# YichengDWu/tinyedm

Hardware: AMD Instinct MI355X
Metric: train imgs/sec CIFAR-10 32x32 bf16 (higher is better)
Workload: dtype bf16; 1 GPU; CIFAR-10 32x32 unconditional EDM2 U-Net (conf/cifar10.yaml, 35.6M params) full training step: diffuse+embed+denoiser fwd/bwd+loss+grad all-reduce+Adam+EMA; per_gpu_batch=128, global_batch=128, parallelism=dp1, conditional=False, step_launch=hipGraph replay, collective=none

## Files before the change

### tinyedm_amd/csrc/tail_lowrank.hip

```cpp
#include "common.h"

typedef __attribute__((ext_vector_type(2))) float f32x2;

constexpr size_t LOWRANK_LDS_MAX = 60 * 1024;
static size_t dgrad_lds(int Co, int C, int W, int R, bool fused) {
  const int CL = C / 8, PS = ((256 / CL) * CL) / CL, TP = (W + 3) / 4 * 4 + 4;
  return ((size_t)Co * 9 * C + (size_t)Co * (R + 2) * TP + (fused ? (size_t)PS * C : 0)) * sizeof(float);
}
static size_t wgrad_lds(int Co, int taps, int C, int W, int R) {
  const int halo = taps == 9 ? 1 : 0;
  return ((size_t)Co * taps * C + (size_t)Co * (R + 2 * halo) * (W + 2 * halo)) * sizeof(float);
}
extern "C" int edm_lowrank_supported(int C, int Co, int W, int taps) {
  if (C <= 0 || C % 8 || C > 1024 || Co < 1 || Co > 8 || W <= 0 || (taps != 1 && taps != 9)) return 0;
  if (wgrad_lds(Co, taps, C, W, 1) > LOWRANK_LDS_MAX) return 0;
  return taps == 1 || dgrad_lds(Co, C, W, 1, true) <= LOWRANK_LDS_MAX;
}

__global__ void k_lowrank_df(const float* __restrict__ dD, const float* __restrict__ Fraw,
                             const float* __restrict__ gain_out, const float* __restrict__ sigma, int sstride, float sd,
                             float* __restrict__ dF, float* __restrict__ aux, int CoHW, long n) {
  const float go = *gain_out;
  for (long i = (long)blockIdx.x * blockDim.x + threadIdx.x; i < n; i += (long)gridDim.x * blockDim.x) {
    const int b = (int)(i / CoHW);
    const float s = sigma[b * sstride];
    const float c = s * sd * rsqrtf(s * s + sd * sd);
    const float d = dD[i];
    dF[i] = d * (c * go);
    if (aux) aux[i] = (d * c) * Fraw[i];
  }
}

extern "C" int edm_lowrank_df(const float* dD, const float* Fraw, const float* gain_out, const float* sigma,
                              int sigma_stride, float sigma_data, float* dF, float* aux, int B, int Co, int HW,
                              hipStream_t st) {
  EDM_REQUIRE(dD && gain_out && sigma && dF && (!aux || Fraw), "lowrank_df: null pointer");
  EDM_REQUIRE(B > 0 && HW > 0 && Co >= 1 && Co <= 8 && (sigma_stride == 0 || sigma_stride == 1), "lowrank_df: bad args");
  EDM_REQUIRE((long)Co * HW < (1L << 31), "lowrank_df: sample too large");
  const long n = (long)B * Co * HW;
  const long blocks = (n + 255) / 256;
  hipLaunchKernelGGL(k_lowrank_df, dim3((unsigned)(blocks < 2048 ? blocks : 2048)), dim3(256), 0, st, dD, Fraw, gain_out,
                     sigma, sigma_stride, sigma_data, dF, aux, Co * HW, n);
  EDM_CHECK_LAUNCH("lowrank_df");
  return EDM_OK;
}

template <int CO, bool FUSED>
__global__ __launch_bounds__(256, 4) void k_lowrank_dgrad3x3(const float* __restrict__ dF, const float* __restrict__ Wc,
                                                          float scale, bf16* __restrict__ ga, const bf16* __restrict__ U,
                                                          const float* __restrict__ lin, long lin_stride,
                                                          const float* __restrict__ gain, bf16* __restrict__ gr,
                                                          float* __restrict__ gm, long gm_stride, float pdrop,
                                                          uint32_t seed_lo, uint32_t seed_hi, uint32_t sub, uint32_t step,
                                                          int u_marks, const StepParams* __restrict__ dyn, int H, int W,
                                                          int C, int R, int TP) {
  extern __shared__ __attribute__((aligned(16))) float sm[];
  float* wl = sm;
  float* tl = wl + CO * 9 * C;
  float* red = tl + CO * (R + 2) * TP;
  const int CL = C >> 3;
  const int PS = blockDim.x / CL;
  const int c8 = threadIdx.x % CL, ps = threadIdx.x / CL;
  const int b = blockIdx.y, y0 = blockIdx.x * R;
  const int rows = min(R, H - y0);
  for (int i = threadIdx.x; i < CO * 9 * C / 4; i += blockDim.x)
    reinterpret_cast<f32x4*>(wl)[i] = reinterpret_cast<const f32x4*>(Wc)[i];
  for (int i = threadIdx.x; i < CO * (R + 2) * TP; i += blockDim.x) {
    const int o = i / ((R + 2) * TP), rem = i - o * (R + 2) * TP;
    const int ry = rem / TP, cx = rem - ry * TP;
    const int y = y0 + ry - 1, x = cx - 1;
    float v = 0.f;
    if (y >= 0 && y < H && x >= 0 && x < W) v = dF[(((long)b * CO + o) * H + y) * W + x];
    tl[i] = v;
  }
  __syncthreads();
  ModEpilogue m{};
  float mv[8], part[8];
  if constexpr (FUSED) {
    m.pdrop = pdrop; m.seed_lo = seed_lo; m.seed_hi = seed_hi; m.sub = sub; m.step = step; m.u_marks = u_marks; m.dyn = dyn;
    apply_dyn(m);
    const float g = *gain;
#pragma unroll
    for (int j = 0; j < 8; ++j) {
      mv[j] = lin[(long)b * lin_stride + c8 * 8 + j] * g + 1.0f;
      part[j] = 0.f;
    }
  }
  const int NSX = (W + 3) >> 2;
  const int nstrips = rows * NSX;
  for (int s = ps; s < nstrips; s += PS) {
    const int ry = s / NSX, x0 = (s - ry * NSX) * 4;
    const long p = ((long)b * H + y0 + ry) * W + x0;
    u32x4 ub[4];
    if constexpr (FUSED) {
#pragma unroll
      for (int k = 0; k < 4; ++k) {
        ub[k] = u32x4{0u, 0u, 0u, 0u};
        if (x0 + k < W) ub[k] = *reinterpret_cast<const u32x4*>(U + (p + k) * C + c8 * 8);
      }
    }
    f32x2 acc[4][4];
#pragma unroll
    for (int k = 0; k < 4; ++k)
#pragma unroll
      for (int j = 0; j < 4; ++j) acc[k][j] = f32x2{0.f, 0.f};
#pragma unroll 1
    for (int g = 0; g < 3 * CO; ++g) {
      const int ky = g / CO, o = g - ky * CO;
      {
        const float* tp = tl + (o * (R + 2) + ry + 2 - ky) * TP + x0;
        float dd[6];
#pragma unroll
        for (int j = 0; j < 6; ++j) dd[j] = tp[j];
#pragma unroll
        for (int kx = 0; kx < 3; ++kx) {
          const float* wp = wl + (o * 9 + ky * 3 + kx) * C + c8 * 8;
          const f32x4 w0 = *reinterpret_cast<const f32x4*>(wp), w1 = *reinterpret_cast<const f32x4*>(wp + 4);
          const f32x2 w[4] = {f32x2{w0[0], w0[1]}, f32x2{w0[2], w0[3]}, f32x2{w1[0], w1[1]}, f32x2{w1[2], w1[3]}};
#pragma unroll
          for (int k = 0; k < 4; ++k) {
            const float d = dd[k + 2 - kx];
            const f32x2 d2 = {d, d};
#pragma unroll
            for (int j = 0; j < 4; ++j) acc[k][j] += d2 * w[j];
          }
        }
      }
    }
    u32x4 o8[4];
#pragma unroll
    for (int k = 0; k < 4; ++k) {
      bf16x8 v;
#pragma unroll
      for (int j = 0; j < 4; ++j) {
        v[2 * j] = (bf16)(scale * acc[k][j][0]);
        v[2 * j + 1] = (bf16)(scale * acc[k][j][1]);
      }
      o8[k] = __builtin_bit_cast(u32x4, v);
    }
#pragma unroll
    for (int k = 0; k < 4; ++k) {
      if (x0 + k < W) {
        const long e = (p + k) * C + c8 * 8;
        if (ga) *reinterpret_cast<u32x4*>(ga + e) = o8[k];
        if constexpr (FUSED) *reinterpret_cast<u32x4*>(gr + e) = mod_silu_drop_bwd8(o8[k], ub[k], e >> 3, mv, m, part);
      }
    }
  }
  if constexpr (FUSED) {
#pragma unroll
    for (int j = 0; j < 8; ++j) red[ps * C + c8 * 8 + j] = part[j];
    __syncthreads();
    for (int c = threadIdx.x; c < C; c += blockDim.x) {
      float s = 0.f;
      for (int q = 0; q < PS; ++q) s += red[q * C + c];
      atomicAdd(gm + (long)b * gm_stride + c, s);
    }
  }
}

template <int CO>
static int launch_dgrad(const float* dF, const float* Wc, float scale, void* ga, const void* U, const float* lin,
                        long lin_stride, const float* gain, void* gr, float* gm, long gm_stride, float pdrop,
                        unsigned long long seed, unsigned sub, unsigned step, int u_marked, int B, int H, int W, int C,
                        const void* dyn, hipStream_t st) {
  const int CL = C / 8, block = (256 / CL) * CL, PS = block / CL;
  const int NSX = (W + 3) / 4, TP = NSX * 4 + 4;
  int R = 128 / W;
  R = R < 1 ? 1 : (R > H ? H : R);
  auto lds = [&](int r) { return dgrad_lds(CO, C, W, r, U != nullptr); };
  while (R > 1 && lds(R) > LOWRANK_LDS_MAX) --R;
  EDM_REQUIRE(lds(R) <= LOWRANK_LDS_MAX, "lowrank_dgrad3x3: Co=%d, C=%d, W=%d need %zu bytes of LDS (60 KB at most)", CO, C, W,
              lds(R));
  const dim3 grid((H + R - 1) / R, B);
  if (U)
    hipLaunchKernelGGL((k_lowrank_dgrad3x3<CO, true>), grid, dim3(block), lds(R), st, dF, Wc, scale, (bf16*)ga,
                       (const bf16*)U, lin, lin_stride, gain, (bf16*)gr, gm, gm_stride, pdrop, (uint32_t)seed,
                       (uint32_t)(seed >> 32), sub, step, u_marked, (const StepParams*)dyn, H, W, C, R, TP);
  else
    hipLaunchKernelGGL((k_lowrank_dgrad3x3<CO, false>), grid, dim3(block), lds(R), st, dF, Wc, scale, (bf16*)ga,
                       (const bf16*)nullptr, (const float*)nullptr, 0L, (const float*)nullptr, (bf16*)nullptr,
                       (float*)nullptr, 0L, 0.f, 0u, 0u, 0u, 0u, 0, (const StepParams*)nullptr, H, W, C, R, TP);
  EDM_CHECK_LAUNCH("lowrank_dgrad3x3");
  return EDM_OK;
}

#define EDM_CO_SWITCH(Co, CALL)      \
  switch (Co) {                      \
    case 1: return CALL(1);          \
    case 2: return CALL(2);          \
    case 3: return CALL(3);          \
    case 4: return CALL(4);          \
    case 5: return CALL(5);          \
    case 6: return CALL(6);          \
    case 7: return CALL(7);          \
    default: return CALL(8);         \
  }

extern "C" int edm_lowrank_dgrad3x3(const float* dF, const float* Wc, float scale, void* ga, const void* r1,
                                    const float* lin, long lin_stride, const float* gain, void* gr, float* gm,
                                    long gm_stride, float pdrop, unsigned long long seed, unsigned sub, unsigned step,
                                    int u_marked, int B, int H, int W, int C, int Co, const void* dyn, hipStream_t st) {
  EDM_REQUIRE(dF && Wc && (ga || r1), "lowrank_dgrad3x3: null pointer");
  EDM_REQUIRE(B > 0 && B <= 65535 && H > 0 && W > 0 && C > 0 && C % 8 == 0 && C <= 2048 && Co >= 1 && Co <= 8,
              "lowrank_dgrad3x3: bad args (C %% 8 == 0, Co <= 8 required)");
  EDM_REQUIRE(((uintptr_t)Wc & 15) == 0, "lowrank_dgrad3x3: Wc must be 16-byte aligned");
  if (r1)
    EDM_REQUIRE(lin && gain && gr && gm && lin_stride >= C && gm_stride >= C && pdrop >= 0.f && pdrop < 1.f,
                "lowrank_dgrad3x3: bad modulation-backward args");
#define CALL(CO_) launch_dgrad<CO_>(dF, Wc, scale, ga, r1, lin, lin_stride, gain, gr, gm, gm_stride, pdrop, seed, sub, step, \
                                    u_marked, B, H, W, C, dyn, st)
  EDM_CO_SWITCH(Co, CALL)
#undef CALL
}

template <int CO, int TAPS, int VEC>
__global__ __launch_bounds__(512) void k_lowrank_wgrad(const float* __restrict__ dF, const bf16* __restrict__ X,
                                                       const float* __restrict__ aux, float* __restrict__ ws, int H,
                                                       int W, int C, int R, int upb, int nunits) {
  constexpr int HALO = TAPS == 9 ? 1 : 0, K = TAPS == 9 ? 3 : 1, NB = 8;
  extern __shared__ __attribute__((aligned(16))) float sm[];
  __shared__ float asums[512];
  const int N = CO * TAPS * C, TPW = W + 2 * HALO, TR = R + 2 * HALO;
  float* accl = sm;
  float* tl = sm + N;
  typedef __attribute__((ext_vector_type(VEC / 2))) unsigned int uraw;
  const int CLV = C / VEC;
  const int PS = blockDim.x / CLV;
  const int cv = threadIdx.x % CLV, ps = threadIdx.x / CLV;
  f32x2 acc[CO * TAPS][VEC / 2];
#pragma unroll
  for (int e = 0; e < CO * TAPS; ++e)
#pragma unroll
    for (int h = 0; h < VEC / 2; ++h) acc[e][h] = f32x2{0.f, 0.f};
  float asum = 0.f;
  for (int u = blockIdx.x; u < nunits; u += gridDim.x) {
    const int b = u / upb, y0 = (u - b * upb) * R;
    const int rows = min(R, H - y0);
    __syncthreads();
    for (int i = threadIdx.x; i < CO * TR * TPW; i += blockDim.x) {
      const int o = i / (TR * TPW), rem = i - o * TR * TPW;
      const int ry = rem / TPW, cx = rem - ry * TPW;
      const int y = y0 + ry - HALO, x = cx - HALO;
      float v = 0.f;
      if (y >= 0 && y < H && x >= 0 && x < W)
        v = dF[(((long)b * CO + o) * H + y) * W + x];
      tl[i] = v;
    }
    if (aux) {
      for (int o = 0; o < CO; ++o) {
        const float* ap = aux + (((long)b * CO + o) * H + y0) * W;
        for (int i = threadIdx.x; i < rows * W; i += blockDim.x) asum += ap[i];
      }
    }
    __syncthreads();
    const int np = rows * W;
    const bf16* xp = X + (((long)b * H + y0) * W) * C + cv * VEC;
    int ry = ps / W, x = ps - (ps / W) * W;
    uraw nx[NB];
    auto fetch = [&](int q0) {
#pragma unroll
      for (int i = 0; i < NB; ++i) {
        const int q = q0 + i * PS;
        nx[i] = uraw{};
        if (q < np) nx[i] = *reinterpret_cast<const uraw*>(xp + (long)q * C);
      }
    };
    fetch(ps);
    for (int q0 = ps; q0 < np; q0 += NB * PS) {
      uraw cur[NB];
#pragma unroll
      for (int i = 0; i < NB; ++i) cur[i] = nx[i];
      if (q0 + NB * PS < np) fetch(q0 + NB * PS);
#pragma unroll
      for (int i = 0; i < NB; ++i) {
        if (q0 + i * PS < np) {
          typedef __attribute__((ext_vector_type(VEC))) __bf16 bfv;
          const bfv xv = __builtin_bit_cast(bfv, cur[i]);
          f32x2 xf[VEC / 2];
#pragma unroll
          for (int h = 0; h < VEC / 2; ++h) xf[h] = f32x2{(float)xv[2 * h], (float)xv[2 * h + 1]};
#pragma unroll
          for (int o = 0; o < CO; ++o)
#pragma unroll
            for (int ky = 0; ky < K; ++ky)
#pragma unroll
              for (int kx = 0; kx < K; ++kx) {
                const float d = tl[(o * TR + ry + 2 * HALO - ky) * TPW + x + 2 * HALO - kx];
                const f32x2 d2 = {d, d};
#pragma unroll
                for (int h = 0; h < VEC / 2; ++h) acc[o * TAPS + ky * K + kx][h] += d2 * xf[h];
              }
        }
        x += PS;
        while (x >= W) {
          x -= W;
          ++ry;
        }
      }
    }
  }
  for (int r = 0; r < PS; ++r) {
    __syncthreads();
    if (ps == r) {
#pragma unroll
      for (int e = 0; e < CO * TAPS; ++e) {
#pragma unroll
        for (int h = 0; h < VEC / 2; ++h) {
          f32x2* ap = reinterpret_cast<f32x2*>(accl + e * C + cv * VEC + 2 * h);
          f32x2 v = acc[e][h];
          if (r) v += *ap;
          *ap = v;
        }
      }
    }
  }
  asums[threadIdx.x] = asum;
  __syncthreads();
  float* row = ws + (long)blockIdx.x * (N + 4);
  for (int i = threadIdx.x; i < N; i += blockDim.x) row[i] = accl[i];
  if (threadIdx.x == 0) {
    float s = 0.f;
    for (int i = 0; i < (int)blockDim.x; ++i) s += asums[i];
    row[N] = s;
  }
}

__global__ __launch_bounds__(1024) void k_lowrank_reduce(const float* __restrict__ ws, int nwg, int N, float* __restrict__ G,
                                                         float* __restrict__ aux_out) {
  __shared__ float part[16][64];
  const int l = threadIdx.x & 63, seg = threadIdx.x >> 6;
  const int e = blockIdx.x * 64 + l;
  const int per = (nwg + 15) / 16;
  const int r0 = seg * per;
  float v[16];
#pragma unroll
  for (int k = 0; k < 16; ++k) {
    const int r = r0 + k;
    v[k] = (e <= N && k < per && r < nwg) ? ws[(long)r * (N + 4) + e] : 0.f;
  }
  float s = 0.f;
#pragma unroll
  for (int k = 0; k < 16; ++k) s += v[k];
  part[seg][l] = s;
  __syncthreads();
  if (seg == 0 && e <= N) {
    float t = 0.f;
#pragma unroll
    for (int k = 0; k < 16; ++k) t += part[k][l];
    if (e < N) G[e] = t;
    else if (aux_out) *aux_out += t;
  }
}

template <int CO>
static int launch_wgrad(const float* dF, const void* X, int taps, const float* aux, float* G, float* aux_out, float* ws,
                        long ws_floats, int B, int H, int W, int C, int nwg, hipStream_t st) {
  constexpr int VEC = CO <= 4 ? 4 : 2;
  const int CLV = C / VEC;
  int PS = 512 / CLV;
  PS = PS > 16 ? 16 : PS;
  const int block = PS * CLV, halo = taps == 9 ? 1 : 0;
  const int N = CO * taps * C;
  int R = 512 / W;
  R = R < 1 ? 1 : (R > H ? H : R);
  auto lds = [&](int r) { return wgrad_lds(CO, taps, C, W, r); };
  while (R > 1 && lds(R) > LOWRANK_LDS_MAX) --R;
  EDM_REQUIRE(lds(R) <= LOWRANK_LDS_MAX, "lowrank_wgrad: Co=%d, taps=%d, C=%d, W=%d need %zu bytes of LDS (60 KB at most)", CO,
              taps, C, W, lds(R));
  const int upb = (H + R - 1) / R;
  EDM_REQUIRE((long)B * upb < (1L << 31), "lowrank_wgrad: too many units");
  const int nunits = B * upb;
  const int grid = nunits < nwg ? nunits : nwg;
  EDM_REQUIRE(ws_floats >= (long)grid * (N + 4), "lowrank_wgrad: workspace of %ld floats, %ld needed", ws_floats,
              (long)grid * (N + 4));
  if (taps == 9)
    hipLaunchKernelGGL((k_lowrank_wgrad<CO, 9, VEC>), dim3(grid), dim3(block), lds(R), st, dF, (const bf16*)X, aux, ws, H, W, C,
                       R, upb, nunits);
  else
    hipLaunchKernelGGL((k_lowrank_wgrad<CO, 1, VEC>), dim3(grid), dim3(block), lds(R), st, dF, (const bf16*)X, aux, ws, H, W, C,
                       R, upb, nunits);
  EDM_CHECK_LAUNCH("lowrank_wgrad");
  hipLaunchKernelGGL(k_lowrank_reduce, dim3((N + 1 + 63) / 64), dim3(1024), 0, st, ws, grid, N, G, aux_out);
  EDM_CHECK_LAUNCH("lowrank_reduce");
  return EDM_OK;
}

constexpr int LOWRANK_WGRAD_NWG = 256;
extern "C" long edm_lowrank_wgrad_workspace(int C, int Co, int taps) {
  return (long)LOWRANK_WGRAD_NWG * ((long)Co * taps * C + 4);
}

extern "C" int edm_lowrank_wgrad(const float* dF, const void* X, int taps, const float* aux, float* G, float* aux_out,
                                 float* ws, long ws_floats, int B, int H, int W, int C, int Co, hipStream_t st) {
  EDM_REQUIRE(dF && X && G && ws && (!aux || aux_out), "lowrank_wgrad: null pointer");
  EDM_REQUIRE(B > 0 && H > 0 && W > 0 && C > 0 && C % 8 == 0 && C <= 1024 && Co >= 1 && Co <= 8 && (taps == 1 || taps == 9),
              "lowrank_wgrad: bad args (C %% 8 == 0, Co <= 8, taps 1 or 9 required)");
#define CALL(CO_) launch_wgrad<CO_>(dF, X, taps, aux, G, aux_out, ws, ws_floats, B, H, W, C, LOWRANK_WGRAD_NWG, st)
  EDM_CO_SWITCH(Co, CALL)
#undef CALL
}

__global__ void k_lowrank_expand_wc(const float* __restrict__ wout, const bf16* __restrict__ wd, float* __restrict__ Wc,
                                    int Co, int O, int I, int taps) {
  const int lane = threadIdx.x & 63;
  const int row = blockIdx.x * (blockDim.x >> 6) + (threadIdx.x >> 6);
  if (row >= taps * I) return;
  const int tt = row / I, ci = row - tt * I;
  float acc[8] = {0, 0, 0, 0, 0, 0, 0, 0};
  for (int c = lane * 8; c < O; c += 64 * 8) {
    float v[8];
    load8(wd + (long)row * O + c, v);
#pragma unroll
    for (int o = 0; o < 8; ++o)
      if (o < Co) {
#pragma unroll
        for (int j = 0; j < 8; ++j) acc[o] += wout[(long)o * O + c + j] * v[j];
      }
  }
#pragma unroll
  for (int o = 0; o < 8; ++o)
    if (o < Co) {
      const float s = wave_sum(acc[o]);
      if (lane == 0) Wc[((long)o * taps + (taps - 1 - tt)) * I + ci] = s;
    }
}
extern "C" int edm_lowrank_expand_wc(const float* wout_hat, const void* wd, float* Wc, int Co, int O, int I, int taps,
                                     hipStream_t st) {
  EDM_REQUIRE(wout_hat && wd && Wc, "lowrank_expand_wc: null pointer");
  EDM_REQUIRE(Co >= 1 && Co <= 8 && O > 0 && O % 8 == 0 && I > 0 && taps >= 1, "lowrank_expand_wc: bad args");
  hipLaunchKernelGGL(k_lowrank_expand_wc, dim3((taps * I + 3) / 4), dim3(256), 0, st, wout_hat, (const bf16*)wd, Wc, Co, O,
                     I, taps);
  EDM_CHECK_LAUNCH("lowrank_expand_wc");
  return EDM_OK;
}

__global__ void k_lowrank_expand_slab(const float* __restrict__ wout, const float* __restrict__ G, float* __restrict__ slab,
                                      float scale, int Co, int O, int I, int Ipad, int taps, long n) {
  for (long e = (long)blockIdx.x * blockDim.x + threadIdx.x; e < n; e += (long)gridDim.x * blockDim.x) {
    const int i = (int)(e % Ipad);
    const long tc = e / Ipad;
    const int c = (int)(tc % O), t = (int)(tc / O);
    float s = 0.f;
    if (i < I)
      for (int o = 0; o < Co; ++o) s += wout[(long)o * O + c] * G[((long)o * taps + t) * I + i];
    slab[e] = scale * s;
  }
}
extern "C" int edm_lowrank_expand_slab(const float* wout_hat, const float* G, float* slab, float scale, int Co, int O, int I,
                                       int Ipad, int taps, hipStream_t st) {
  EDM_REQUIRE(wout_hat && G && slab, "lowrank_expand_slab: null pointer");
  EDM_REQUIRE(Co >= 1 && Co <= 8 && O > 0 && I > 0 && Ipad >= I && taps >= 1, "lowrank_expand_slab: bad args");
  const long n = (long)taps * O * Ipad;
  const long blocks = (n + 255) / 256;
  hipLaunchKernelGGL(k_lowrank_expand_slab, dim3((unsigned)(blocks < 4096 ? blocks : 4096)), dim3(256), 0, st, wout_hat, G,
                     slab, scale, Co, O, I, Ipad, taps, n);
  EDM_CHECK_LAUNCH("lowrank_expand_slab");
  return EDM_OK;
}

constexpr int TAIL_LPP = 8;
static size_t tail_fwd_lds(int Co, int C, int Cc, int W, int R) {
  return ((size_t)Co * 9 * C + (size_t)Co * Cc + (size_t)R * W * 10 * Co) * sizeof(float);
}
extern "C" int edm_lowrank_tail_supported(int C, int Cc, int Co, int W) {
  if (C <= 0 || C % 8 || C > 1024 || Cc <= 0 || Cc % 8 || Cc > 2048 || Co < 1 || Co > 8 || W <= 0) return 0;
  return tail_fwd_lds(Co, C, Cc, W, 1) <= LOWRANK_LDS_MAX;
}

template <int CO, int NK, int PX>
__device__ __forceinline__ void tail_dots(const bf16* const (&xp)[PX], int Cx, const float* __restrict__ w, int wso, int lig,
                                          float (&s)[PX][NK * CO]) {
  f32x2 acc[PX][NK * CO];
#pragma unroll
  for (int k = 0; k < PX; ++k)
#pragma unroll
    for (int v = 0; v < NK * CO; ++v) acc[k][v] = f32x2{0.f, 0.f};
  const int CL = Cx >> 3;
  for (int c8 = lig; c8 < CL; c8 += TAIL_LPP) {
    f32x2 xf[PX][4];
#pragma unroll
    for (int k = 0; k < PX; ++k) {
      u32x4 raw = u32x4{0u, 0u, 0u, 0u};
      if (xp[k]) raw = *reinterpret_cast<const u32x4*>(xp[k] + c8 * 8);
      const bf16x8 xv = __builtin_bit_cast(bf16x8, raw);
#pragma unroll
      for (int h = 0; h < 4; ++h) xf[k][h] = f32x2{(float)xv[2 * h], (float)xv[2 * h + 1]};
    }
#pragma unroll
    for (int o = 0; o < CO; ++o)
#pragma unroll
      for (int kk = 0; kk < NK; ++kk) {
        const float* wp = w + (long)(o * wso + kk) * Cx + c8 * 8;
        const f32x4 w0 = *reinterpret_cast<const f32x4*>(wp), w1 = *reinterpret_cast<const f32x4*>(wp + 4);
        const f32x2 wv[4] = {f32x2{w0[0], w0[1]}, f32x2{w0[2], w0[3]}, f32x2{w1[0], w1[1]}, f32x2{w1[2], w1[3]}};
#pragma unroll
        for (int k = 0; k < PX; ++k)
#pragma unroll
          for (int h = 0; h < 4; ++h) acc[k][kk * CO + o] += xf[k][h] * wv[h];
      }
  }
#pragma unroll
  for (int k = 0; k < PX; ++k)
#pragma unroll
    for (int v = 0; v < NK * CO; ++v) s[k][v] = group_sum<TAIL_LPP>(acc[k][v][0] + acc[k][v][1]);
}

template <int CO, int PX>
__global__ __launch_bounds__(512) void k_lowrank_tail_fwd(const bf16* __restrict__ a2, const bf16* __restrict__ cat,
                                                          const float* __restrict__ Wc, const float* __restrict__ Wp,
                                                          float sb, float sa, const float* __restrict__ gain_out,
                                                          const float* __restrict__ noisy, const float* __restrict__ sigma,
                                                          int sstride, float sd, float* __restrict__ D,
                                                          float* __restrict__ Fraw, int H, int W, int C, int Cc, int R) {
  extern __shared__ __attribute__((aligned(16))) float sm[];
  float* wl = sm;
  float* wpl = wl + CO * 9 * C;
  float* pt = wpl + CO * Cc;
  const int RW = R * W;
  float* qt = pt + 3 * RW * 3 * CO;
  const int b = blockIdx.y, y0 = blockIdx.x * R;
  const int rows = min(R, H - y0);
  for (int i = threadIdx.x; i < CO * 9 * C / 4; i += blockDim.x)
    reinterpret_cast<f32x4*>(wl)[i] = reinterpret_cast<const f32x4*>(Wc)[i];
  for (int i = threadIdx.x; i < CO * Cc / 4; i += blockDim.x)
    reinterpret_cast<f32x4*>(wpl)[i] = reinterpret_cast<const f32x4*>(Wp)[i];
  __syncthreads();
  const int lig = threadIdx.x % TAIL_LPP, grp = threadIdx.x / TAIL_LPP, NG = blockDim.x / TAIL_LPP;
#pragma unroll 1
  for (int ky = 0; ky < 3; ++ky) {
    const int r_lo = max(y0 + ky - 1, 0), r_hi = min(y0 + rows - 1 + ky - 1, H - 1);
    const int np = (r_hi - r_lo + 1) * W;
    const int slot0 = (r_lo - (y0 + ky - 1)) * W;
    const bf16* base = a2 + (((long)b * H + r_lo) * W) * C;
    float* po = pt + (long)ky * RW * 3 * CO;
    for (int n0 = grp * PX; n0 < np; n0 += NG * PX) {
      const bf16* xp[PX];
#pragma unroll
      for (int k = 0; k < PX; ++k) xp[k] = n0 + k < np ? base + (long)(n0 + k) * C : nullptr;
      float s[PX][3 * CO];
      tail_dots<CO, 3, PX>(xp, C, wl + ky * 3 * C, 9, lig, s);
#pragma unroll
      for (int k = 0; k < PX; ++k)
        if (n0 + k < np) {
#pragma unroll
          for (int v = 0; v < 3 * CO; ++v)
            if ((v % TAIL_LPP) == lig) po[(long)(slot0 + n0 + k) * 3 * CO + v] = s[k][v];
        }
    }
  }
  {
    const int np = rows * W;
    const bf16* base = cat + (((long)b * H + y0) * W) * Cc;
    for (int n0 = grp * PX; n0 < np; n0 += NG * PX) {
      const bf16* xp[PX];
#pragma unroll
      for (int k = 0; k < PX; ++k) xp[k] = n0 + k < np ? base + (long)(n0 + k) * Cc : nullptr;
      float s[PX][CO];
      tail_dots<CO, 1, PX>(xp, Cc, wpl, 1, lig, s);
#pragma unroll
      for (int k = 0; k < PX; ++k)
        if (n0 + k < np) {
#pragma unroll
          for (int v = 0; v < CO; ++v)
            if ((v % TAIL_LPP) == lig) qt[(long)(n0 + k) * CO + v] = s[k][v];
        }
    }
  }
  __syncthreads();
  const float go = *gain_out;
  const float sg = sigma[b * sstride];
  const float den = sg * sg + sd * sd;
  const float cskip = sd * sd / den, cout = sg * sd * rsqrtf(den);
  for (int i = threadIdx.x; i < CO * rows * W; i += blockDim.x) {
    const int o = i / (rows * W), n = i - o * rows * W;
    const int ry = n / W, x = n - ry * W;
    float s = 0.f;
#pragma unroll
    for (int ky = 0; ky < 3; ++ky) {
      const int iy = y0 + ry + ky - 1;
      if (iy < 0 || iy >= H) continue;
#pragma unroll
      for (int kx = 0; kx < 3; ++kx) {
        const int ix = x + kx - 1;
        if (ix < 0 || ix >= W) continue;
        s += pt[((long)ky * RW + ry * W + ix) * 3 * CO + kx * CO + o];
      }
    }
    const float f = sb * s + sa * qt[(long)n * CO + o];
    const long idx = (((long)b * CO + o) * H + y0 + ry) * W + x;
    if (Fraw) Fraw[idx] = f;
    D[idx] = f * go * cout + noisy[idx] * cskip;
  }
}

template <int CO>
static int launch_tail_fwd(const void* a2, const void* cat, const float* Wc, const float* Wp, float sb, float sa,
                           const float* gain_out, const float* noisy, const float* sigma, int sstride, float sd, float* D,
                           float* Fraw, int B, int H, int W, int C, int Cc, hipStream_t st) {
  constexpr int PX = CO <= 4 ? 2 : 1;
  int R = 128 / W;
  R = R < 1 ? 1 : (R > H ? H : R);
  auto lds = [&](int r) { return tail_fwd_lds(CO, C, Cc, W, r); };
  while (R > 1 && lds(R) > LOWRANK_LDS_MAX) --R;
  EDM_REQUIRE(lds(R) <= LOWRANK_LDS_MAX, "lowrank_tail_fwd: Co=%d, C=%d, Cc=%d, W=%d need %zu bytes of LDS (60 KB at most)", CO,
              C, Cc, W, lds(R));
  const long want = ((long)(R + 1) * W + PX - 1) / PX * TAIL_LPP;
  int block = want >= 512 ? 512 : (int)((want + 63) / 64 * 64);
  const dim3 grid((H + R - 1) / R, B);
  hipLaunchKernelGGL((k_lowrank_tail_fwd<CO, PX>), grid, dim3(block), lds(R), st, (const bf16*)a2, (const bf16*)cat, Wc, Wp, sb,
                     sa, gain_out, noisy, sigma, sstride, sd, D, Fraw, H, W, C, Cc, R);
  EDM_CHECK_LAUNCH("lowrank_tail_fwd");
  return EDM_OK;
}

extern "C" int edm_lowrank_tail_fwd(const void* a2, const void* cat, const float* Wc, const float* Wp, float sb, float sa,
                                    const float* gain_out, const float* noisy, const float* sigma, int sigma_stride,
                                    float sigma_data, float* D, float* Fraw, int B, int H, int W, int C, int Cc, int Co,
                                    hipStream_t st) {
  EDM_REQUIRE(a2 && cat && Wc && Wp && gain_out && noisy && sigma && D, "lowrank_tail_fwd: null pointer");
  EDM_REQUIRE(B > 0 && B <= 65535 && H > 0 && W > 0 && (sigma_stride == 0 || sigma_stride == 1), "lowrank_tail_fwd: bad args");
  EDM_REQUIRE(edm_lowrank_tail_supported(C, Cc, Co, W), "lowrank_tail_fwd: unsupported shape C=%d Cc=%d Co=%d W=%d", C, Cc, Co, W);
  EDM_REQUIRE((((uintptr_t)Wc | (uintptr_t)Wp | (uintptr_t)a2 | (uintptr_t)cat) & 15) == 0,
              "lowrank_tail_fwd: operands must be 16-byte aligned");
#define CALL(CO_) launch_tail_fwd<CO_>(a2, cat, Wc, Wp, sb, sa, gain_out, noisy, sigma, sigma_stride, sigma_data, D, Fraw, B, \
                                       H, W, C, Cc, st)
  EDM_CO_SWITCH(Co, CALL)
#undef CALL
}

__global__ __launch_bounds__(256) void k_lowrank_tail_dwout(const float* __restrict__ G, const bf16* __restrict__ wf2,
                                                            const float* __restrict__ G1, const bf16* __restrict__ wf1,
                                                            float sb, float sa, float* __restrict__ gwh, int Co, int C,
                                                            int Cc) {
  const int lane = threadIdx.x & 63;
  const int c = blockIdx.x * (blockDim.x >> 6) + (threadIdx.x >> 6);
  if (c >= C) return;
  float a9[8] = {0, 0, 0, 0, 0, 0, 0, 0}, a1[8] = {0, 0, 0, 0, 0, 0, 0, 0};
  for (int t = 0; t < 9; ++t)
    for (int ci = lane * 8; ci < C; ci += 64 * 8) {
      float v[8];
      load8(wf2 + ((long)t * C + c) * C + ci, v);
#pragma unroll
      for (int o = 0; o < 8; ++o)
        if (o < Co) {
          const float* gp = G + ((long)o * 9 + t) * C + ci;
#pragma unroll
          for (int j = 0; j < 8; ++j) a9[o] += v[j] * gp[j];
        }
    }
  if (wf1)
    for (int cj = lane * 8; cj < Cc; cj += 64 * 8) {
      float v[8];
      load8(wf1 + (long)c * Cc + cj, v);
#pragma unroll
      for (int o = 0; o < 8; ++o)
        if (o < Co) {
          const float* gp = G1 + (long)o * Cc + cj;
#pragma unroll
          for (int j = 0; j < 8; ++j) a1[o] += v[j] * gp[j];
        }
    }
#pragma unroll
  for (int o = 0; o < 8; ++o)
    if (o < Co) {
      const float s9 = wave_sum(a9[o]);
      const float s1 = wf1 ? wave_sum(a1[o]) : G1[(long)o * Cc + c];
      if (lane == 0) gwh[(long)o * C + c] = sb * s9 + sa * s1;
    }
}
extern "C" int edm_lowrank_tail_dwout_supported(int C, int Cc, int Co, int has1) {
  return C > 0 && C % 8 == 0 && Cc > 0 && Cc % 8 == 0 && Co >= 1 && Co <= 8 && (has1 || Cc == C);
}
extern "C" int edm_lowrank_tail_dwout(const float* G, const void* wf2, const float* G1, const void* wf1, float sb, float sa,
                                      float* gwh, int Co, int C, int Cc, hipStream_t st) {
  EDM_REQUIRE(G && wf2 && G1 && gwh, "lowrank_tail_dwout: null pointer");
  EDM_REQUIRE(edm_lowrank_tail_dwout_supported(C, Cc, Co, wf1 != nullptr), "lowrank_tail_dwout: bad args (C=%d Cc=%d Co=%d)", C, Cc,
              Co);
  EDM_REQUIRE((((uintptr_t)wf2 | (uintptr_t)wf1) & 15) == 0, "lowrank_tail_dwout: packs must be 16-byte aligned");
  hipLaunchKernelGGL(k_lowrank_tail_dwout, dim3((C + 3) / 4), dim3(256), 0, st, G, (const bf16*)wf2, G1, (const bf16*)wf1, sb,
                     sa, gwh, Co, C, Cc);
  EDM_CHECK_LAUNCH("lowrank_tail_dwout");
  return EDM_OK;
}

__global__ void k_lowrank_gcat_add(const float* __restrict__ dF, const float* __restrict__ Wp, float sa,
                                   const bf16* __restrict__ t, bf16* __restrict__ gu, bf16* __restrict__ gcs, int HW, int Cc,
                                   int Ci, int Co, long n8) {
  const unsigned CL = (unsigned)Cc >> 3, uHW = (unsigned)HW, CiL = (unsigned)Ci >> 3;
  for (unsigned i = blockIdx.x * blockDim.x + threadIdx.x; i < (unsigned)n8; i += gridDim.x * blockDim.x) {
    const unsigned p = i / CL, c8 = i - p * CL;
    const unsigned b = p / uHW, hw = p - b * uHW;
    float v[8] = {0, 0, 0, 0, 0, 0, 0, 0}, tv[8];
    load8(t + (long)i * 8, tv);
    for (int o = 0; o < Co; ++o) {
      const float df = dF[((long)b * Co + o) * HW + hw];
      const float* wp = Wp + (long)o * Cc + c8 * 8;
#pragma unroll
      for (int j = 0; j < 8; ++j) v[j] += df * wp[j];
    }
#pragma unroll
    for (int j = 0; j < 8; ++j) v[j] = tv[j] + sa * v[j];
    if (c8 < CiL) store8(gu + ((long)p * Ci + c8 * 8), v);
    else store8(gcs + ((long)p * (Cc - Ci) + (c8 - CiL) * 8), v);
  }
}
extern "C" int edm_lowrank_gcat_supported(int Cc, int Ci, int Co) {
  return Cc > 0 && Cc % 8 == 0 && Ci > 0 && Ci % 8 == 0 && Ci <= Cc && Co >= 1 && Co <= 8;
}
extern "C" int edm_lowrank_gcat_add(const float* dF, const float* Wp, float sa, const void* t, void* gu, void* gcs, int B,
                                    int HW, int Cc, int Ci, int Co, hipStream_t st) {
  EDM_REQUIRE(dF && Wp && t && gu, "lowrank_gcat_add: null pointer");
  EDM_REQUIRE(B > 0 && HW > 0 && edm_lowrank_gcat_supported(Cc, Ci, Co) && (gcs || Ci == Cc),
              "lowrank_gcat_add: bad args (Cc=%d Ci=%d Co=%d)", Cc, Ci, Co);
  const long n8 = (long)B * HW * (Cc / 8);
  EDM_REQUIRE(n8 < (1L << 31), "lowrank_gcat_add: too many elements");
  const long blocks = (n8 + 255) / 256;
  hipLaunchKernelGGL(k_lowrank_gcat_add, dim3((unsigned)(blocks < 8192 ? blocks : 8192)), dim3(256), 0, st, dF, Wp, sa,
                     (const bf16*)t, (bf16*)gu, (bf16*)gcs, HW, Cc, Ci, Co, n8);
  EDM_CHECK_LAUNCH("lowrank_gcat_add");
  return EDM_OK;
}
```

Measured before the change: 10480 img/s.

## Add MFMA-based low-rank 3x3 weight-gradient kernel with async LDS ring pipeline

Adds a new kernel for the low-rank tail's 3x3 weight gradient, used when the output has at most 3 channels. It computes the reduction over pixels with bf16 MFMA 32x32x16. The fp32 dF tap images are split into three bf16 terms (hi, mid, lo) to keep near-fp32 accuracy. Activations are streamed through a multi-stage LDS ring with global_load_lds DMA and read back with transpose reads. It replaces a scalar/vector FMA path, at the cost of three MFMAs per block, more LDS and an env-var gated code path.

```diff
diff --git a/tinyedm_amd/csrc/tail_lowrank.hip b/tinyedm_amd/csrc/tail_lowrank.hip
--- a/tinyedm_amd/csrc/tail_lowrank.hip
+++ b/tinyedm_amd/csrc/tail_lowrank.hip
@@ -1,4 +1,5 @@
 #include "common.h"
+#include <stdlib.h>
 
 typedef __attribute__((ext_vector_type(2))) float f32x2;
 
@@ -353,9 +354,228 @@
   }
 }
 
+namespace {
+typedef const __attribute__((address_space(1))) void* lr_gptr_t;
+typedef __attribute__((address_space(3))) void* lr_lptr_t;
+typedef __attribute__((address_space(3))) char lr_lds_char;
+__device__ __forceinline__ void lr_dma16(const void* src, char* lds_dst) {
+  __builtin_amdgcn_global_load_lds((lr_gptr_t)src, (lr_lptr_t)lds_dst, 16, 0, 0);
+}
+template <int N>
+__device__ __forceinline__ void lr_wait_vm(int n) {
+  if constexpr (N == 0) {
+    asm volatile("s_waitcnt vmcnt(0)" ::: "memory");
+  } else {
+    if (n >= N) asm volatile("s_waitcnt vmcnt(%0)" ::"n"(N) : "memory");
+    else lr_wait_vm<N - 1>(n);
+  }
+}
+#define LR_TR_RD(dst, base, imm) asm volatile("ds_read_b64_tr_b16 %0, %1 offset:%2" : "=v"(dst) : "v"(base), "i"(imm))
+__device__ __forceinline__ bf16x8 lr_frag(const u32x2& lo, const u32x2& hi) {
+  u32x4 v = __builtin_shufflevector(lo, hi, 0, 1, 2, 3);
+  return __builtin_bit_cast(bf16x8, v);
+}
+constexpr int LR_MAXB = 4;
+constexpr size_t LOWRANK_MFMA_LDS_MAX = 144 * 1024;
+}
+
+template <int CO>
+__global__ __launch_bounds__(512) void k_lowrank_wgrad_mfma(const float* __restrict__ dF, const bf16* __restrict__ X,
+                                                            const float* __restrict__ aux, float* __restrict__ ws,
+                                                            const bf16* __restrict__ zeros, int H, int W, int C, int R,
+                                                            int upb, int nunits, int ring) {
+  constexpr int TAPS = 9, HALO = 1, K = 3, NT = CO * TAPS;
+  static_assert(NT <= 32, "the rows of G must fit one MFMA block");
+  extern __shared__ __attribute__((aligned(16))) char smem[];
+  __shared__ float asums[512];
+  const int tid = threadIdx.x, lane = tid & 63, NW = blockDim.x >> 6;
+  const int wave = __builtin_amdgcn_readfirstlane(tid >> 6);
+  const int nblk = C >> 5, stageB = C * 64, slotB = stageB + 3 * 2048;
+  const int NI = 2 * nblk / NW;
+  float* tl = reinterpret_cast<float*>(smem + ring * slotB);
+  const int TPW = W + 2 * HALO, TR = R + 2 * HALO;
+  int nbw = 0;
+#pragma unroll
+  for (int i = 0; i < LR_MAXB; ++i)
+    if (wave + i * NW < nblk) nbw = i + 1;
+  f32x16 acc[LR_MAXB];
+#pragma unroll
+  for (int i = 0; i < LR_MAXB; ++i)
+#pragma unroll
+    for (int r = 0; r < 16; ++r) acc[i][r] = 0.f;
+  const int krow_l = 8 * (lane >> 5) + ((lane & 15) >> 2);
+  const int chan_b = (16 * ((lane >> 4) & 1) + 4 * (lane & 3)) * 2;
+  const unsigned lds0 = (unsigned)(uintptr_t)(lr_lds_char*)smem + krow_l * 64 + chan_b;
+  float asum = 0.f;
+  for (int u = blockIdx.x; u < nunits; u += gridDim.x) {
+    const int b = u / upb, y0 = (u - b * upb) * R;
+    const int rows = min(R, H - y0);
+    const int np = rows * W, nst = (np + 31) >> 5;
+    const bf16* xu = X + (((long)b * H + y0) * W) * C;
+    auto issue = [&](int t) {
+      char* dst = smem + (t % ring) * slotB;
+      for (int i = 0; i < NI; ++i) {
+        const int j = wave + NW * i;
+        const int row = t * 32 + (j & 1) * 16 + (lane >> 2);
+        const bf16* src = row < np ? xu + (long)row * C + (j >> 1) * 32 + (lane & 3) * 8 : zeros;
+        lr_dma16(src, dst + (j >> 1) * 2048 + (j & 1) * 1024);
+      }
+    };
+    auto images = [&](int t) {
+      char* img = smem + (t % ring) * slotB + stageB;
+      for (int i = tid; i < 32 * 16; i += blockDim.x) {
+        const int q = t * 32 + (i >> 4), cp = (i & 15) * 2;
+        const int ry = q / W, x = q - ry * W;
+        bf16x2 part[3];
+#pragma unroll
+        for (int e = 0; e < 2; ++e) {
+          const int n = cp + e;
+          float d = 0.f;
+          if (q < np && n < NT) {
+            const int o = n / TAPS, tp = n - o * TAPS;
+            const int ky = tp / K, kx = tp - ky * K;
+            d = tl[(o * TR + ry + 2 * HALO - ky) * TPW + x + 2 * HALO - kx];
+          }
+          part[0][e] = (bf16)d;
+          const float r1 = d - (float)part[0][e];
+          part[1][e] = (bf16)r1;
+          part[2][e] = (bf16)(r1 - (float)part[1][e]);
+        }
+#pragma unroll
+        for (int g = 0; g < 3; ++g) *reinterpret_cast<bf16x2*>(img + g * 2048 + (i >> 4) * 64 + cp * 2) = part[g];
+      }
+    };
+    __syncthreads();
+    const int pre = min(ring - 1, nst);
+    for (int t = 0; t < pre; ++t) issue(t);
+    for (int i = tid; i < CO * TR * TPW; i += blockDim.x) {
+      const int o = i / (TR * TPW), rem = i - o * TR * TPW;
+      const int ry = rem / TPW, cx = rem - ry * TPW;
+      const int y = y0 + ry - HALO, x = cx - HALO;
+      float v = 0.f;
+      if (y >= 0 && y < H && x >= 0 && x < W) v = dF[(((long)b * CO + o) * H + y) * W + x];
+      tl[i] = v;
+    }
+    if (aux) {
+      for (int o = 0; o < CO; ++o) {
+        const float* ap = aux + (((long)b * CO + o) * H + y0) * W;
+        for (int i = tid; i < np; i += blockDim.x) asum += ap[i];
+      }
+    }
+    __syncthreads();
+    for (int t = 0; t < pre; ++t) images(t);
+    for (int t = 0; t < nst; ++t) {
+      const int last = min(t + ring - 2, nst - 1);
+      lr_wait_vm<24>(__builtin_amdgcn_readfirstlane(NI * (last - t)));
+      asm volatile("s_waitcnt lgkmcnt(0)" ::: "memory");
+      __builtin_amdgcn_s_barrier();
+      if (t + ring - 1 < nst) {
+        issue(t + ring - 1);
+        images(t + ring - 1);
+      }
+      const unsigned sb = lds0 + (t % ring) * slotB;
+      const unsigned ah = sb + stageB;
+      if (nbw > 0) {
+#pragma unroll
+        for (int ks = 0; ks < 2; ++ks) {
+          u32x2 a0, a1, m0, m1, l0, l1, x0[LR_MAXB], x1[LR_MAXB];
+          LR_TR_RD(a0, ah, ks * 1024);
+          LR_TR_RD(a1, ah, ks * 1024 + 256);
+          LR_TR_RD(m0, ah, 2048 + ks * 1024);
+          LR_TR_RD(m1, ah, 2048 + ks * 1024 + 256);
+          LR_TR_RD(l0, ah, 4096 + ks * 1024);
+          LR_TR_RD(l1, ah, 4096 + ks * 1024 + 256);
+#pragma unroll
+          for (int i = 0; i < LR_MAXB; ++i)
+            if (i < nbw) {
+              const unsigned xb = sb + (wave + i * NW) * 2048;
+              LR_TR_RD(x0[i], xb, ks * 1024);
+              LR_TR_RD(x1[i], xb, ks * 1024 + 256);
+            }
+          asm volatile("s_waitcnt lgkmcnt(0)" ::: "memory");
+          __builtin_amdgcn_sched_barrier(0);
+#pragma unroll
+          for (int i = 0; i < LR_MAXB; ++i)
+            if (i < nbw) {
+              acc[i] = __builtin_amdgcn_mfma_f32_32x32x16_bf16(lr_frag(l0, l1), lr_frag(x0[i], x1[i]), acc[i], 0, 0, 0);
+              acc[i] = __builtin_amdgcn_mfma_f32_32x32x16_bf16(lr_frag(m0, m1), lr_frag(x0[i], x1[i]), acc[i], 0, 0, 0);
+              acc[i] = __builtin_amdgcn_mfma_f32_32x32x16_bf16(lr_frag(a0, a1), lr_frag(x0[i], x1[i]), acc[i], 0, 0, 0);
+            }
+          __builtin_amdgcn_sched_barrier(0);
+        }
+      }
+    }
+  }
+  const int N = NT * C, l31 = lane & 31, lhi = lane >> 5;
+  float* row = ws + (long)blockIdx.x * (N + 4);
+#pragma unroll
+  for (int i = 0; i < LR_MAXB; ++i)
+    if (i < nbw) {
+      const int c = (wave + i * NW) * 32 + l31;
+#pragma unroll
+      for (int r = 0; r < 16; ++r) {
+        const int n = (r & 3) + 8 * (r >> 2) + 4 * lhi;
+        if (n < NT) row[(long)n * C + c] = acc[i][r];
+      }
+    }
+  asums[tid] = asum;
+  __syncthreads();
+  if (tid == 0) {
+    float s = 0.f;
+    for (int i = 0; i < (int)blockDim.x; ++i) s += asums[i];
+    row[N] = s;
+  }
+}
+
+static bool lowrank_mfma_on() {
+  const char* e = getenv("EDM_LOWRANK_MFMA");
+  return !(e && e[0] == '0');
+}
+struct WgradMfmaPlan {
+  int R, ring, NW;
+  size_t lds;
+};
+static bool wgrad_mfma_plan(int Co, int taps, int C, int H, int W, const void* X, WgradMfmaPlan& p) {
+  if (taps != 9 || !lowrank_mfma_on() || C % 32 || Co * 9 + Co > 32 || W > 64 || ((uintptr_t)X & 15)) return false;
+  const int nblk = C / 32, halo = 1;
+  p.NW = (2 * nblk) % 8 == 0 ? 8 : ((2 * nblk) % 4 == 0 ? 4 : 2);
+  if ((nblk + p.NW - 1) / p.NW > LR_MAXB) return false;
+  const size_t slot = (size_t)C * 64 + 3 * 2048;
+  int R = 512 / W;
+  R = R < 1 ? 1 : (R > H ? H : R);
+  auto tile = [&](int r) { return (size_t)Co * (r + 2 * halo) * (W + 2 * halo) * sizeof(float); };
+  while (R > 1 && tile(R) + 2 * slot > LOWRANK_MFMA_LDS_MAX) --R;
+  if (tile(R) + 2 * slot > LOWRANK_MFMA_LDS_MAX) return false;
+  const size_t ring = (LOWRANK_MFMA_LDS_MAX - tile(R)) / slot;
+  p.R = R;
+  const int NI = 2 * nblk / p.NW, most = 2 + 24 / NI;
+  p.ring = (int)ring > (most < 6 ? most : 6) ? (most < 6 ? most : 6) : (int)ring;
+  p.lds = tile(R) + p.ring * slot;
+  return true;
+}
+
 template <int CO>
 static int launch_wgrad(const float* dF, const void* X, int taps, const float* aux, float* G, float* aux_out, float* ws,
                         long ws_floats, int B, int H, int W, int C, int nwg, hipStream_t st) {
+  if constexpr (CO <= 3) {
+    WgradMfmaPlan p;
+    if (wgrad_mfma_plan(CO, taps, C, H, W, X, p)) {
+      EDM_ZERO_PAGE(zeros, "lowrank_wgrad");
+      const int N = CO * taps * C, upb = (H + p.R - 1) / p.R;
+      EDM_REQUIRE((long)B * upb < (1L << 31), "lowrank_wgrad: too many units");
+      const int nunits = B * upb;
+      const int grid = nunits < nwg ? nunits : nwg;
+      EDM_REQUIRE(ws_floats >= (long)grid * (N + 4), "lowrank_wgrad: workspace of %ld floats, %ld needed", ws_floats,
+                  (long)grid * (N + 4));
+      EDM_MAX_LDS((k_lowrank_wgrad_mfma<CO>), (int)LOWRANK_MFMA_LDS_MAX);
+      hipLaunchKernelGGL((k_lowrank_wgrad_mfma<CO>), dim3(grid), dim3(p.NW * 64), p.lds, st, dF, (const bf16*)X, aux, ws,
+                         (const bf16*)zeros, H, W, C, p.R, upb, nunits, p.ring);
+      EDM_CHECK_LAUNCH("lowrank_wgrad (mfma)");
+      hipLaunchKernelGGL(k_lowrank_reduce, dim3((N + 1 + 63) / 64), dim3(1024), 0, st, ws, grid, N, G, aux_out);
+      EDM_CHECK_LAUNCH("lowrank_reduce");
+      return EDM_OK;
+    }
+  }
   constexpr int VEC = CO <= 4 ? 4 : 2;
   const int CLV = C / VEC;
   int PS = 512 / CLV;
```

Result: no change. 10470 img/s (-0.1%).
